# biotite-dev/springcraft

Measured on AMD Instinct MI355X. Metric: ANM modes/sec (Hessian build + full eigensolve), N=2000 C-alpha, higher is better.
Workload: dtype f64; 1 GPU; C3: N=2000 C-alpha ANM, HinsenForceField (no cutoff), full 6000x6000 eigensolve, all modes + vectors; parallelism=independent structures sharded over GPUs, no data-path collective

## Files before the change

### springcraft_amd/csrc/api.hip

```cpp
#include <algorithm>
#include <cmath>
#include <cstdarg>
#include <cstring>
#include <map>
#include <new>
#include <utility>

#include "common.h"
#include "host_logic.h"

int sc_set_error(sc_ctx* ctx, int code, const char* fmt, ...) {
  char buf[1024];
  va_list ap;
  va_start(ap, fmt);
  vsnprintf(buf, sizeof(buf), fmt, ap);
  va_end(ap);
  if (ctx) ctx->err = buf;
  return code;
}

static int reserve(sc_ctx* ctx, void*& buf, size_t& have, size_t bytes, bool collect_events = false) {
  if (bytes <= have) return SC_OK;
  if (buf) {
    SC_HIP(ctx, hipStreamSynchronize(ctx->stream));
// ... 326 lines not shown
}

const char* sc_last_error(sc_ctx* ctx) { return ctx ? ctx->err.c_str() : "null context"; }

int sc_host_alloc(size_t bytes, void** out) {
  if (!out || bytes == 0) return SC_ERR_INVALID_ARG;
  *out = nullptr;
  void* p = nullptr;
  if (hipHostMalloc(&p, bytes, hipHostMallocDefault) != hipSuccess || !p) {
    (void)hipGetLastError();
    return SC_ERR_NOMEM;
  }
  *out = p;
  return SC_OK;
}

int sc_host_free(void* p) {
  if (!p) return SC_OK;
  return hipHostFree(p) == hipSuccess ? SC_OK : SC_ERR_HIP;
}

int sc_ctx_synchronize(sc_ctx* ctx) {
  if (!ctx) return SC_ERR_INVALID_ARG;
  SC_HIP(ctx, hipSetDevice(ctx->device));
  SC_HIP(ctx, hipStreamSynchronize(ctx->stream));
  return sc_deferred_status(ctx);
}

int sc_device_info(sc_ctx* ctx, char* buf, size_t buflen) {
  if (!ctx || !buf || buflen == 0) return SC_ERR_INVALID_ARG;
  hipDeviceProp_t prop;
  SC_HIP(ctx, hipGetDeviceProperties(&prop, ctx->device));
  snprintf(buf, buflen, "%s %s, %d CUs, %.0f GiB", prop.gcnArchName, prop.name,
           prop.multiProcessorCount, (double)prop.totalGlobalMem / (1 << 30));
  return SC_OK;
}

int sc_ctx_set_profiling(sc_ctx* ctx, int enabled) {
  if (!ctx) return SC_ERR_INVALID_ARG;
  ctx->profiling = enabled != 0;
  return SC_OK;
}

int sc_last_eigh_timings(sc_ctx* ctx, double* out6) {
  if (!ctx || !out6) return SC_ERR_INVALID_ARG;
  for (int i = 0; i < 6; ++i) out6[i] = ctx->last_timings[i];
  return SC_OK;
}

int sc_last_eigh_phase_ms(sc_ctx* ctx, const char* name, double* ms) {
  if (!ctx || !name || !ms) return SC_ERR_INVALID_ARG;
  for (const auto& p : ctx->phases)
    if (p.first == name) { *ms = p.second; return SC_OK; }
  *ms = 0.0;
  return SC_ERR_INVALID_ARG;
}

int sc_ctx_get_counter(sc_ctx* ctx, const char* name, int64_t* value) {
  if (!ctx || !name || !value) return SC_ERR_INVALID_ARG;
  const std::string k(name);
  SC_HIP(ctx, hipSetDevice(ctx->device));
  SC_HIP(ctx, hipStreamSynchronize(ctx->stream));
  SC_TRY(sc_collect_events(ctx));
  int tmin = ctx->chase_tickets[0], tmax = ctx->chase_tickets[0];
  long long tsum = 0;
  for (int x = 0; x < std::max(1, std::min(8, ctx->chase_ctl_xcds)); ++x) {
    tmin = std::min(tmin, ctx->chase_tickets[x]);
    tmax = std::max(tmax, ctx->chase_tickets[x]);
    tsum += ctx->chase_tickets[x];
  }
  if (k == "chase_launches") *value = ctx->cnt_chase_launches;
  else if (k == "chase_pair_launches") *value = ctx->cnt_pair_launches;
  else if (k == "chase_pair_fallbacks") *value = ctx->cnt_pair_fallbacks;
  else if (k == "xcd_count") *value = ctx->nxcd;
  else if (k == "gemm3_launches") *value = ctx->cnt_gemm3_launches;
  else if (k == "symm3_launches") *value = ctx->cnt_symm3_launches;
  else if (k == "resident_launches") *value = ctx->cnt_resident_launches;
  else if (k == "resident_takeovers") *value = ctx->cnt_resident_takeovers;
  else if (k == "resident_rollcall_failures") *value = ctx->cnt_resident_rollcalls;
  else if (k == "resident_lost_waits") *value = ctx->cnt_resident_lost;
  else if (k == "resident_lost_at") *value = ctx->resident_lost_at;
  else if (k == "panel_coop_launches") *value = ctx->cnt_coop_launches;
  else if (k == "panel_coop_timeouts") *value = ctx->cnt_coop_timeouts;
  else if (k == "chase_timeouts") *value = ctx->cnt_chase_timeouts;
  else if (k == "chase_incomplete") *value = ctx->cnt_chase_incomplete;
  else if (k == "chase_resumed") *value = ctx->cnt_chase_resumed;
  else if (k == "chase_sweeps") *value = ctx->cnt_chase_sweeps;
  else if (k == "stepwise_chases") *value = ctx->cnt_stepwise_chases;
  else if (k == "chase_xcd_min") *value = tmin;
  else if (k == "chase_xcd_max") *value = tmax;
  else if (k == "chase_xcd_total") *value = tsum;
  else if (k == "chase_wait_matrix") *value = ctx->chase_wait[0];
  else if (k == "chase_wait_sweep") *value = ctx->chase_wait[1];
  else if (k == "chase_wait_task") *value = ctx->chase_wait[2];
  else { *value = 0; return SC_ERR_INVALID_ARG; }
  return SC_OK;
}

int sc_dbg_set_chase(sc_ctx* ctx, int mode, int give_up_after) {
  if (!ctx || mode < -1 || mode > 5 || give_up_after < 0) return SC_ERR_INVALID_ARG;
  ctx->chase_form = mode == 3 ? 1 : (mode == 4 ? 0 : (mode == 5 ? 2 : -1));
  if (mode > 2) mode = 2;
  ctx->chase_mode = mode;
  ctx->chase_give_up = give_up_after;
  if (mode >= 0) ctx->chase_ok = -1;
  return SC_OK;
}

int sc_dbg_set_panel_coop_fail(sc_ctx* ctx, int panel) {
  if (!ctx || panel < -1) return SC_ERR_INVALID_ARG;
  ctx->coop_fail_panel = panel;
  if (panel >= 0) ctx->coop_ok = -1;
  return SC_OK;
}

int sc_dbg_set_resident(sc_ctx* ctx, int mode, int hook, int workgroups) {
  if (!ctx || mode < -1 || mode > 1 || hook < 0 || workgroups < 0 || workgroups > 256) return SC_ERR_INVALID_ARG;
  ctx->resident_mode = mode;
  ctx->resident_hook = hook;
  ctx->resident_wgs = workgroups;
  if (mode != 0) { ctx->resident_ok = -1; ctx->resident_strikes = 0; }
  return SC_OK;
}

int sc_dbg_set_panel_coop(sc_ctx* ctx, int min_rows) {
  if (!ctx || min_rows < -1 || (min_rows > 0 && min_rows < 128)) return SC_ERR_INVALID_ARG;
  ctx->coop_min_rows = min_rows;
  if (min_rows != 0) ctx->coop_ok = -1;
  return SC_OK;
}

int sc_contacts(sc_ctx* ctx, const double* coord, int64_t n, const sc_ff_desc* ff,
                const sc_patch_desc* patch, int64_t* counts, int64_t* n_pairs) {
  SC_TRY(check_coord_args(ctx, coord, n));
  SC_TRY(check_ff(ctx, ff));
  SC_HIP(ctx, hipSetDevice(ctx->device));
  if (n_pairs) *n_pairs = 0;
  if (n == 0) return SC_OK;
  Staged st;
  Bump bump{};
  SC_TRY(stage_inputs(ctx, coord, n, ff, patch, nullptr, (size_t)n * 8 + 256, st, bump));
  int64_t* d_counts = bump.take<int64_t>((size_t)n);
  SC_TRY(launch_contact_counts(ctx, st.d_coord, n, st.ff_dev, st.has_patch ? &st.patch : nullptr, d_counts));
  std::vector<int64_t> h((size_t)n);
  SC_HIP(ctx, hipMemcpyAsync(h.data(), d_counts, (size_t)n * 8, hipMemcpyDeviceToHost, ctx->stream));
  SC_HIP(ctx, hipStreamSynchronize(ctx->stream));
  int64_t total = 0;
  for (int64_t i = 0; i < n; ++i) total += h[(size_t)i];
  if (counts) std::memcpy(counts, h.data(), (size_t)n * 8);
  if (n_pairs) *n_pairs = total;
  return SC_OK;
}

int sc_pairs(sc_ctx* ctx, const double* coord, int64_t n, const sc_ff_desc* ff,
             const sc_patch_desc* patch, int64_t capacity, int64_t* pairs, double* sq_dist,
             int64_t* n_pairs) {
  SC_TRY(check_coord_args(ctx, coord, n));
  SC_TRY(check_ff(ctx, ff));
  if (capacity < 0 || (capacity > 0 && !pairs))
    return sc_set_error(ctx, SC_ERR_INVALID_ARG, "pairs buffer is NULL");
  SC_HIP(ctx, hipSetDevice(ctx->device));
  if (n_pairs) *n_pairs = 0;
  if (n == 0) return SC_OK;
  Staged st;
  Bump bump{};
  const size_t extra = (size_t)(2 * n + 2) * 8 + (size_t)capacity * 24 + 2048;
// ... 1107 lines not shown
```

### springcraft_amd/csrc/common.h

```cpp
#pragma once

#include <hip/hip_runtime.h>

#include <cstdint>
#include <cstdio>
#include <map>
#include <mutex>
#include <string>
#include <utility>
#include <vector>

#include "../../include/springcraft_hip.h"

struct sc_ctx {
  int device = 0;
  hipStream_t stream = nullptr;
  bool own_stream = false;
  hipStream_t aux_stream = nullptr;
  std::vector<hipStream_t> side_streams;
  std::vector<hipEvent_t> side_joins;
  hipEvent_t aux_fork = nullptr, aux_join = nullptr;
  std::string err;
  int num_cus = 0;

  void* ws = nullptr;
  size_t ws_bytes = 0;
  void* scratch = nullptr;
  size_t scratch_bytes = 0;
  void* dc_aux = nullptr;
  size_t dc_aux_bytes = 0;
  void* pinv_ws = nullptr;
  size_t pinv_ws_bytes = 0;
  void* win_ws = nullptr;
  size_t win_ws_bytes = 0;
  void* modes_ws = nullptr;
  size_t modes_ws_bytes = 0;

  char* h_stage[2] = {nullptr, nullptr};
  size_t h_stage_bytes[2] = {0, 0}, h_stage_off[2] = {0, 0};
  hipEvent_t h_stage_done[2] = {nullptr, nullptr};
  bool h_stage_pending[2] = {false, false};
  int h_stage_cur = 0;
  unsigned long long* d_status = nullptr;

  int two_stage = -1;
  int chase_ok = -1;
  int chase_mode = -1, chase_give_up = 0;
  int chase_form = -1;
  int nxcd = 0;
  int pair_attr = -1;
  long long cnt_pair_fallbacks = 0;
  int gemm3_attr = -1;
  void* d_zeros = nullptr;
  long long cnt_symm3_launches = 0;
  bool gemm3_side_by_side = false;
  long long cnt_gemm3_launches = 0;
  int coop_attr = -1, coop_ok = -1;
  int coop_min_rows = -1;
  int coop_fail_panel = -1;
  int resident_ok = -1, resident_mode = -1, resident_hook = 0, resident_wgs = 0;
  long long cnt_resident_launches = 0, cnt_resident_takeovers = 0, cnt_resident_rollcalls = 0, cnt_resident_lost = 0;
  long long resident_lost_at = -1;
  int resident_strikes = 0;
  int* d_chase_ctl = nullptr;
  int* last_chase_ctl = nullptr;
  int chase_ctl_xcds = 8;
  long long cnt_coop_launches = 0, cnt_coop_timeouts = 0;
  long long cnt_chase_launches = 0, cnt_chase_timeouts = 0, cnt_chase_incomplete = 0, cnt_chase_resumed = 0,
            cnt_chase_sweeps = 0, cnt_stepwise_chases = 0, cnt_pair_launches = 0;
  int chase_tickets[8] = {0, 0, 0, 0, 0, 0, 0, 0};
  int chase_wait[3] = {-1, -1, -1};
  bool profiling = false;
  double last_timings[6] = {0, 0, 0, 0, 0, 0};
  std::vector<std::pair<std::string, double>> phases;
};

class PhaseTimer {
 public:
  PhaseTimer(sc_ctx* ctx, const char* name, hipStream_t st) : ctx_(ctx), name_(name), st_(st), on_(ctx->profiling) {}
  ~PhaseTimer() { for (hipEvent_t e : ev_) (void)hipEventDestroy(e); }
  void start() { mark(); }
  void stop() { mark(); }
  void finish() {
    if (!on_ || ev_.size() < 2) return;
    double total = 0.0;
    if (hipEventSynchronize(ev_.back()) != hipSuccess) return;
    for (size_t i = 0; i + 1 < ev_.size(); i += 2) {
      float ms = 0.f;
      if (hipEventElapsedTime(&ms, ev_[i], ev_[i + 1]) == hipSuccess) total += ms;
    }
    for (auto& p : ctx_->phases)
      if (p.first == name_) { p.second = total; return; }
    ctx_->phases.emplace_back(name_, total);
  }
 private:
  void mark() {
    if (!on_) return;
    hipEvent_t e = nullptr;
    if (hipEventCreate(&e) != hipSuccess) { on_ = false; return; }
    (void)hipEventRecord(e, st_);
    ev_.push_back(e);
  }
  sc_ctx* ctx_;
  std::string name_;
  hipStream_t st_;
  bool on_;
  std::vector<hipEvent_t> ev_;
};

template <int N>
struct ScopedEvents {
  hipEvent_t e[N];
  ScopedEvents() { for (auto& x : e) x = nullptr; }
  ~ScopedEvents() { for (auto& x : e) if (x) (void)hipEventDestroy(x); }
  ScopedEvents(const ScopedEvents&) = delete;
  ScopedEvents& operator=(const ScopedEvents&) = delete;
  hipEvent_t& operator[](int i) { return e[i]; }
  hipEvent_t* begin() { return e; }
  hipEvent_t* end() { return e + N; }
};

int sc_set_error(sc_ctx* ctx, int code, const char* fmt, ...);

#define SC_HIP(ctx, call)                                                              \
  do {                                                                                 \
    hipError_t e__ = (call);                                                           \
    if (e__ != hipSuccess)                                                             \
      return sc_set_error((ctx), e__ == hipErrorOutOfMemory ? SC_ERR_NOMEM : SC_ERR_HIP, \
                          "%s failed: %s (%s:%d)", #call, hipGetErrorString(e__),      \
                          __FILE__, __LINE__);                                         \
  } while (0)

#define SC_TRY(expr)            \
  do {                          \
    int rc__ = (expr);          \
    if (rc__ != SC_OK) return rc__; \
  } while (0)

int sc_reserve_ws(sc_ctx* ctx, size_t bytes);
int sc_reserve_scratch(sc_ctx* ctx, size_t bytes);
int sc_reserve_dc_aux(sc_ctx* ctx, size_t bytes);
int sc_reserve_pinv(sc_ctx* ctx, size_t bytes);
int sc_reserve_win(sc_ctx* ctx, size_t bytes);
int sc_reserve_modes(sc_ctx* ctx, size_t bytes);
int sc_aux_stream(sc_ctx* ctx);
int sc_side_streams(sc_ctx* ctx, int count);
int sc_stage_upload(sc_ctx* ctx, void* d_dst, const void* h_src, size_t bytes);
int sc_stage_end(sc_ctx* ctx);
constexpr int kSpStatusWords = 16;
constexpr int kChaseCtlInts = 32;
// ... 108 lines not shown
```

### springcraft_amd/csrc/sy2sb.hip

```cpp
#include <algorithm>
#include <vector>

#include "twostage_internal.h"

namespace {

constexpr int kEarly = (kIb + 2) / 2;

__global__ __launch_bounds__(256) void k_panel_qr(double* __restrict__ a_all, long long stride_a,
                                                  double* __restrict__ tri_all, TriLayout TL,
                                                  double* __restrict__ sb_all, SbLayout SL, int j0, int j, int nr,
                                                  int c_end) {
  constexpr int LD = kQrRows + 1;
  extern __shared__ __attribute__((aligned(16))) double sm[];
  const int c_lo = j > 0 ? j - 1 : 0;
  const int ncl = c_end - c_lo;
  double* P = sm;
  double* wv = sm + ncl * LD;
  double* vv = wv + kB;
  double* red = vv + kQrRows;
  __shared__ double s_scale, s_beta, s_tau;

  const int n = TL.n;
  const int r0 = j0 + kB, m = n - r0;
// ... 852 lines not shown
                                                       double* __restrict__ sb_all, SbLayout SL, int j0,
                                                       const int* __restrict__ ctl, unsigned long long* __restrict__ stats) {
  __shared__ double red[16 * 9];
  __shared__ double s_w[8];
  __shared__ double s_tau, s_beta, s_scale;
  const int mat = blockIdx.x;
  if (ctl[8 * mat] == 0) return;
  const int n = TL.n;
  const int r0 = j0 + kB, m = n - r0;
  double* A = a_all + (size_t)mat * stride_a;
  double* tri = tri_all + (size_t)mat * TL.slab;
  double* sb = sb_all + (size_t)mat * SL.slab;
  double* P = A + (size_t)j0 * n + r0;
  const int tid = threadIdx.x, lane = tid & 63, wv = tid >> 6;
  if (tid == 0) atomicAdd(stats + 5, 1ull);
  auto block_sum8 = [&](double (&a)[8], int cnt) {
    for (int i = 0; i < cnt; ++i) {
      const double t = wave_sum(a[i]);
      if (lane == 0) red[wv * 9 + i] = t;
    }
    __syncthreads();
    for (int i = 0; i < cnt; ++i) {
      double t = 0.0;
      for (int w = 0; w < 16; ++w) t += red[w * 9 + i];
      a[i] = t;
    }
    __syncthreads();
  };
  for (int j = 0; j < kB; ++j) {
    double* pj = P + (size_t)j * n;
    {
      double a[8] = {0, 0, 0, 0, 0, 0, 0, 0};
      for (int r = j + 1 + tid; r < m; r += 1024) a[0] += pj[r] * pj[r];
      block_sum8(a, 1);
      if (tid == 0) {
        const HH h = householder(pj[j], a[0]);
        s_tau = h.tau; s_beta = h.beta; s_scale = h.scale;
        tri[TL.tau + j0 + j] = h.tau;
      }
      __syncthreads();
    }
    const double tau = s_tau, scale = s_scale;
    for (int c0 = j + 1; c0 < kB; c0 += 8) {
      const int cnt = min(8, kB - c0);
      double a[8] = {0, 0, 0, 0, 0, 0, 0, 0};
      for (int r = j + 1 + tid; r < m; r += 1024) {
        const double x = pj[r];
        for (int i = 0; i < cnt; ++i) a[i] += x * P[(size_t)(c0 + i) * n + r];
      }
      block_sum8(a, cnt);
      if (tid < cnt) s_w[tid] = tau * (P[(size_t)(c0 + tid) * n + j] + scale * a[tid]);
      __syncthreads();
      for (int r = j + tid; r < m; r += 1024) {
        const double v = r > j ? scale * pj[r] : 1.0;
        for (int i = 0; i < cnt; ++i) P[(size_t)(c0 + i) * n + r] -= v * s_w[i];
      }
      __syncthreads();
    }
    for (int r = j + tid; r < m; r += 1024) pj[r] = r > j ? scale * pj[r] : s_beta;
    __syncthreads();
  }
  for (int c = 0; c < kB; ++c)
    for (int r = tid; r < m; r += 1024) {
      const double val = P[(size_t)c * n + r];
      const double v = r > c ? val : (r == c ? 1.0 : 0.0);
      sb[SL.vw + (size_t)c * n + r0 + r] = v;
      sb[SL.wv + (size_t)(kB + c) * n + r0 + r] = -v;
      sb[SL.xv + (size_t)(2 * kB + c) * n + r0 + r] = v;
    }
}

__global__ __launch_bounds__(256) void k_sum_xslices(double* __restrict__ sb_all, SbLayout SL, int r0) {
  const int n = SL.n, p = SL.symm_split;
  double* sb = sb_all + (size_t)blockIdx.z * SL.slab;
  const int which = blockIdx.y / kB, c = blockIdx.y % kB;
  const int r = r0 + blockIdx.x * 256 + threadIdx.x;
  if (r >= n) return;
  const double* src = sb + SL.xsplit + (size_t)which * p * n * kB + (size_t)c * n + r;
  double s = 0.0;
  for (int q = 0; q < p; ++q) s += src[(size_t)q * n * kB];
  sb[SL.xv + (size_t)(which * kB + c) * n + r] = s;
}

__global__ __launch_bounds__(256) void k_sum_p2(double* __restrict__ sb_all, SbLayout SL) {
  double* sb = sb_all + (size_t)blockIdx.y * SL.slab;
  const int i = blockIdx.x * 256 + threadIdx.x;
  double acc = 0.0;
#pragma unroll
  for (int sl = 0; sl < kSmallSplit; ++sl) acc += sb[SL.small2 + (size_t)sl * 2 * kB * kB + i];
  sb[SL.p2 + i] = acc;
}

__global__ __launch_bounds__(1024) void k_sb_small(const double* __restrict__ tri_all, TriLayout TL,
                                                   double* __restrict__ sb_all, SbLayout SL, int j0) {
  constexpr int LD = kB + 1;
  extern __shared__ __attribute__((aligned(16))) double sm[];
  double* G = sm;
  double* M1 = G + kB * LD;
  double* T = M1 + kB * LD;
  double* U = T + kB * LD;
  const double* tri = tri_all + (size_t)blockIdx.x * TL.slab;
  double* sb = sb_all + (size_t)blockIdx.x * SL.slab;
  const int tid = threadIdx.x, nthr = blockDim.x;
  const double* prod = sb + SL.small;
  const size_t slice = (size_t)kB * 3 * kB;
  for (int idx = tid; idx < kB * kB; idx += nthr) {
    const int i = idx & 63, jj = idx >> 6;
    double g = 0.0, x = 0.0;
#pragma unroll
    for (int s = 0; s < kSmallSplit; ++s) {
      const double* ps = prod + s * slice;
      x += ps[i + (size_t)jj * kB] + ps[i + (size_t)(kB + jj) * kB];
      g += ps[i + (size_t)(2 * kB + jj) * kB];
    }
    G[i * LD + jj] = g;
    M1[i * LD + jj] = x;
    T[i * LD + jj] = 0.0;
  }
  __syncthreads();
  if (tid < kB) {
    const int bb = tid >> 4, c = tid & 15, o = bb * 16;
    double x[16];
#pragma unroll
    for (int i = 15; i >= 0; --i) {
      double acc = (i == c) ? 1.0 : 0.0;
#pragma unroll
      for (int l = i + 1; l < 16; ++l) acc -= G[(o + i) * LD + o + l] * x[l];
      x[i] = i <= c ? tri[TL.tau + j0 + o + i] * acc : 0.0;
    }
#pragma unroll
    for (int i = 0; i < 16; ++i) T[(o + i) * LD + o + c] = x[i];
  }
  __syncthreads();
#pragma unroll
  for (int bs = 16; bs <= 32; bs *= 2) {
    const int npair = kB / (2 * bs);
    for (int idx = tid; idx < npair * bs * bs; idx += nthr) {
      const int pr = idx / (bs * bs), e = idx % (bs * bs), i = e / bs, jj = e % bs;
      const int o1 = pr * 2 * bs, o2 = o1 + bs;
      double acc = 0.0;
      for (int l = 0; l <= jj; ++l) acc += G[(o1 + i) * LD + o2 + l] * T[(o2 + l) * LD + o2 + jj];
      U[(o1 + i) * LD + o2 + jj] = acc;
    }
    __syncthreads();
    for (int idx = tid; idx < npair * bs * bs; idx += nthr) {
      const int pr = idx / (bs * bs), e = idx % (bs * bs), i = e / bs, jj = e % bs;
      const int o1 = pr * 2 * bs, o2 = o1 + bs;
      double acc = 0.0;
      for (int l = i; l < bs; ++l) acc += T[(o1 + i) * LD + o1 + l] * U[(o1 + l) * LD + o2 + jj];
      T[(o1 + i) * LD + o2 + jj] = -acc;
    }
    __syncthreads();
  }
  for (int idx = tid; idx < kB * kB; idx += nthr) {
    const int i = idx >> 6, jj = idx & 63;
    double s = 0.0;
    for (int l = 0; l <= jj; ++l) s += M1[i * LD + l] * T[l * LD + jj];
    U[i * LD + jj] = s;
  }
  __syncthreads();
  double* cm = sb + SL.cmat;
  for (int idx = tid; idx < kB * kB; idx += nthr) {
    const int i = idx & 63, jj = idx >> 6;
    double s = 0.0;
    for (int l = 0; l <= i; ++l) s += T[l * LD + i] * U[l * LD + jj];
    const double t = T[i * LD + jj];
    cm[i + (size_t)jj * 3 * kB] = t;
    cm[kB + i + (size_t)jj * 3 * kB] = t;
    cm[2 * kB + i + (size_t)jj * 3 * kB] = -0.5 * s;
  }
}

}


std::vector<GemmDesc> sb_stage1_records(int n, int batch, const std::vector<int>& role, double* d_a, long long stride_a,
                                        double* d_sb_ws, const SbLayout& SL) {
  const sc_host::TwoStageEnv& E = sc_host::two_stage_env();
  const int npanels = (int)role.size();
  std::vector<GemmDesc> h((size_t)npanels * kDescKinds * batch);
  for (int p = 0; p < npanels; ++p) {
    const int j0 = p * kB, r0 = j0 + kB, m = n - r0;
    const int rl = role[(size_t)p];
    const long long vw_w = rl == 2 ? 3 * kB : kB, wv_w = rl == 2 ? 2 * kB : 0;
    for (int b = 0; b < batch; ++b) {
      double* A = d_a + (size_t)b * stride_a;
      double* sb = d_sb_ws + (size_t)b * SL.slab;
      double* a22 = A + (size_t)r0 * n + r0;
      GemmDesc* g = &h[((size_t)p * batch + b) * kDescKinds];
      GemmDesc X1{};
      X1.a = a22; X1.sa_i = 1; X1.sa_k = n; X1.a_tri = 1;
      X1.b = sb + SL.xv + (size_t)2 * kB * n + r0; X1.sb_k = 1; X1.sb_j = n;
      X1.c = sb + SL.xv + r0; X1.ldc = n;
      X1.m = m; X1.n = kB; X1.k = m; X1.alpha = 1.0; X1.beta = 0.0;
      if (SL.symm_split > 1) {
        X1.c = sb + SL.xsplit + r0;
        X1.split_stride = (long long)n * kB;
      }
      g[0] = X1;
      GemmDesc X2 = X1;
      X2.sa_i = n; X2.sa_k = 1; X2.a_tri = 2;
      X2.c = sb + SL.xv + (size_t)kB * n + r0;
      if (SL.symm_split > 1) X2.c = sb + SL.xsplit + (size_t)SL.symm_split * n * kB + r0;
      g[1] = X2;
      GemmDesc P{};
      P.a = sb + SL.xv + (size_t)2 * kB * n + r0; P.sa_i = n; P.sa_k = 1;
      P.b = sb + SL.xv + r0; P.sb_k = 1; P.sb_j = n;
      P.c = sb + SL.small; P.ldc = kB;
      P.m = kB; P.n = 3 * kB; P.k = m; P.alpha = 1.0; P.beta = 0.0;
      P.split_stride = (long long)kB * 3 * kB;
      g[2] = P;
      GemmDesc W{};
      W.a = sb + SL.xv + r0; W.sa_i = 1; W.sa_k = n;
      W.b = sb + SL.cmat; W.sb_k = 1; W.sb_j = 3 * kB;
      W.c = sb + SL.vw + (size_t)vw_w * n + r0; W.ldc = n;
      W.m = m; W.n = kB; W.k = 3 * kB; W.alpha = 1.0; W.beta = 0.0;
      g[3] = W;
      W.c = sb + SL.wv + (size_t)wv_w * n + r0;
      W.alpha = -1.0;
      g[4] = W;
      GemmDesc R{};
      R.a = sb + SL.vw + r0; R.sa_i = 1; R.sa_k = n;
      R.b = sb + SL.wv + r0; R.sb_k = n; R.sb_j = 1;
      R.c = a22; R.ldc = n;
      R.m = m; R.n = m; R.k = rl == 2 ? 4 * kB : 2 * kB; R.alpha = 1.0; R.beta = 1.0;
      R.lower_only = sc_host::symm3_for(E, n) ? 2 : 1;
      g[5] = R;
      GemmDesc D = R;
      D.n = kB; D.k = 2 * kB;
      g[6] = D;
      GemmDesc Q{};
      Q.a = sb + SL.wv + r0; Q.sa_i = n; Q.sa_k = 1;
      Q.b = sb + SL.xv + (size_t)2 * kB * n + r0; Q.sb_k = 1; Q.sb_j = n;
      Q.c = sb + SL.small2; Q.ldc = 2 * kB;
      Q.m = 2 * kB; Q.n = kB; Q.k = m; Q.alpha = 1.0; Q.beta = 0.0;
      Q.split_stride = (long long)2 * kB * kB;
      g[7] = Q;
      GemmDesc Cr{};
      Cr.a = sb + SL.vw + r0; Cr.sa_i = 1; Cr.sa_k = n;
      Cr.b = sb + SL.p2; Cr.sb_k = 1; Cr.sb_j = 2 * kB;
      Cr.c = sb + SL.xv + r0; Cr.ldc = n;
      Cr.m = m; Cr.n = kB; Cr.k = 2 * kB; Cr.alpha = 1.0; Cr.beta = 1.0;
      g[8] = Cr;
    }
  }
  std::vector<GemmDesc> hs(h.size());
  for (int p = 0; p < npanels; ++p)
    for (int b = 0; b < batch; ++b) {
      const GemmDesc* g = &h[((size_t)p * batch + b) * kDescKinds];
      GemmDesc* o = &hs[(size_t)p * kDescKinds * batch];
      for (int kd = 0; kd < kDescKinds; ++kd) o[(size_t)kd * batch + b] = g[kd];
    }
  return hs;
}

struct PanelRun {
  sc_ctx* ctx;
  hipStream_t st;
  double* d_a; long long stride_a; int n, batch;
  double* d_tri_ws; const TriLayout& TL;
  double* d_sb_ws; const SbLayout& SL;
  const GemmDesc* d_descs;
  const std::vector<int>& role;
  sc_host::CoopPlan coop;
  v4i* coop_recs;
  int* coop_ctl;
  bool use_symm3;
  int symm3_nb_min;
  SbTimers& t;
};

static int run_panel(const PanelRun& R, int p, int lo, int hi, hipStream_t ps, bool timed) {
  using sc_host::PanelQr;
  const sc_host::TwoStageEnv& E = sc_host::two_stage_env();
  sc_ctx* ctx = R.ctx;
  const TriLayout& TL = R.TL;
  const SbLayout& SL = R.SL;
  const int n = R.n, batch = R.batch;
  const long long stride_a = R.stride_a;
  struct StreamScope {
    sc_ctx* c; hipStream_t old;
    StreamScope(sc_ctx* c_, hipStream_t s) : c(c_), old(c_->stream) { c->stream = s; }
    ~StreamScope() { c->stream = old; }
  } scope(ctx, ps);
  const int nb = hi - lo;
  const int rl = R.role[(size_t)p];
  double* a_h = R.d_a + (size_t)lo * stride_a;
  double* tri_h = R.d_tri_ws + (size_t)lo * TL.slab;
  double* sb_h = R.d_sb_ws + (size_t)lo * SL.slab;
  const int j0 = p * kB, r0 = j0 + kB, m = n - r0;
  const int nr = std::min(kB, m - 1);
  const int nchunks = (m + kQrRows - 1) / kQrRows;
  const dim3 qgrid((unsigned)nchunks, (unsigned)nb);
  SbLayout SQ = SL;
  if (rl == 2) { SQ.vw += (long long)2 * kB * n; SQ.wv += (long long)2 * kB * n; }
  if (timed) R.t.qr.start();
  const sc_host::PanelQrForm F = sc_host::panel_qr_form(E, R.coop, R.coop_recs != nullptr, m, nb, ps == R.st);
  switch (F.kind) {
    case PanelQr::Coop: {
      const int coop_g = F.coop_g;
      if (p == ctx->coop_fail_panel) SC_HIP(ctx, hipMemsetAsync(R.coop_ctl + 8 * lo, 1, sizeof(int) * 8 * nb, ps));
      hipLaunchKernelGGL(k_panel_coop, dim3((unsigned)coop_g, (unsigned)nb), dim3(kCoopRows), kCoopLdsBytes, ps, a_h, stride_a,
                         tri_h, TL, sb_h, SQ, j0, coop_g, R.coop_recs + (size_t)lo * coop_recs_per_matrix(coop_g),
                         R.coop_ctl + 8 * lo, (p + 1) * 128);
      hipLaunchKernelGGL(k_panel_serial, dim3((unsigned)nb), dim3(1024), 0, ps, a_h, stride_a, tri_h, TL, sb_h, SQ, j0,
                         (const int*)(R.coop_ctl + 8 * lo), ctx->d_status);
      ++ctx->cnt_coop_launches;
      break;
    }
    case PanelQr::Wg1024: {
      const size_t lds_wg = sizeof(double) * (size_t)(2 * kWgWaves * 8 + 16 + 8 + 8 * kB + kWgWaves * kB * 8);
      const dim3 g1((unsigned)nb), b1((unsigned)kWgThreads);
      if (F.ru == 1) hipLaunchKernelGGL((k_panel_wg<1, 8>), g1, b1, lds_wg, ps, a_h, stride_a, tri_h, TL, sb_h, SQ, j0);
      else if (F.ru == 2) hipLaunchKernelGGL((k_panel_wg<2, 8>), g1, b1, lds_wg, ps, a_h, stride_a, tri_h, TL, sb_h, SQ, j0);
      else if (F.ru == 3) hipLaunchKernelGGL((k_panel_wg<3, 4>), g1, b1, lds_wg, ps, a_h, stride_a, tri_h, TL, sb_h, SQ, j0);
      else hipLaunchKernelGGL((k_panel_wg<4, 2>), g1, b1, lds_wg, ps, a_h, stride_a, tri_h, TL, sb_h, SQ, j0);
      break;
    }
    case PanelQr::Wg512: {
      constexpr int kW = 512 / 64;
      const size_t lds_wg = sizeof(double) * (size_t)(2 * kW * 8 + 16 + 8 + 8 * kB + kW * kB * 8);
      const dim3 g1((unsigned)nb), b1(512u);
      if (F.ru == 10) hipLaunchKernelGGL((k_panel_wg<10, 1, 512>), g1, b1, lds_wg, ps, a_h, stride_a, tri_h, TL, sb_h, SQ, j0);
      else hipLaunchKernelGGL((k_panel_wg<12, 1, 512>), g1, b1, lds_wg, ps, a_h, stride_a, tri_h, TL, sb_h, SQ, j0);
      break;
    }
    case PanelQr::Blocked: {
      const size_t lds_qr_blk = sizeof(double) * ((size_t)(kIb + 1) * (kQrRows + 1) + kB + kQrRows + 4 * kB);
      const size_t lds_blk_a = sizeof(double) * ((size_t)kB * (kQrRows + 1) + kQrRows + 8 * kB);
      const size_t lds_blk_b = sizeof(double) * ((size_t)kB * (kQrRows + 1) + kIb * kB + 4 * kB);
      hipLaunchKernelGGL(k_panel_qr, qgrid, dim3(256), lds_qr_blk, ps, a_h, stride_a, tri_h, TL, sb_h, SQ, j0, 0, nr, kIb);
      for (int c0 = 0; c0 < kB; c0 += kIb) {
        for (int j = c0 + 1; j < c0 + kIb; ++j)
          hipLaunchKernelGGL(k_panel_qr, qgrid, dim3(256), lds_qr_blk, ps, a_h, stride_a, tri_h, TL, sb_h, SQ, j0, j, nr,
                             c0 + kIb);
        const size_t cut = sizeof(double) * (size_t)c0 * (kQrRows + 1);
        hipLaunchKernelGGL(k_pqr_blk_a, qgrid, dim3(256), lds_blk_a - cut, ps, a_h, stride_a, tri_h, TL, sb_h, SQ, j0, c0);
        if (c0 + kIb < kB)
          hipLaunchKernelGGL(k_pqr_blk_b, qgrid, dim3(256), lds_blk_b - cut, ps, a_h, stride_a, tri_h, TL, sb_h, SQ, j0, c0);
      }
      break;
    }
    case PanelQr::Unblocked: {
      const size_t lds_qr = sizeof(double) * ((size_t)kB * (kQrRows + 1) + kB + kQrRows + 4 * kB);
      for (int j = 0; j <= nr; ++j)
        hipLaunchKernelGGL(k_panel_qr, qgrid, dim3(256), lds_qr, ps, a_h, stride_a, tri_h, TL, sb_h, SQ, j0, j, nr, kB);
      break;
    }
  }
  if (timed) R.t.qr.stop();
  const GemmDesc* g = R.d_descs + (size_t)p * kDescKinds * batch;
  if (timed) R.t.symm.start();
  if (R.use_symm3 && symm3_would_take(ctx, R.symm3_nb_min, m, SL.symm_split, true) &&
      launch_symm3(ctx, g + lo, nb, m, SL.symm_split, true, true) == SC_OK) {
    if (SL.symm_split > 1)
      hipLaunchKernelGGL(k_sum_xslices, dim3((unsigned)((m + 255) / 256), kB, (unsigned)nb), dim3(256), 0, ps, sb_h, SL, r0);
  } else {
    SC_TRY(launch_gemm_f64(ctx, g + lo, nb, m, kB, kGemmTile, SL.symm_split, false, true, kGemmAmBk));
    SC_TRY(launch_gemm_f64(ctx, g + batch + lo, nb, m, kB, kGemmTile, SL.symm_split, false, true, kGemmAkBk));
    if (SL.symm_split > 1)
      hipLaunchKernelGGL(k_sum_xslices, dim3((unsigned)((m + 255) / 256), 2 * kB, (unsigned)nb), dim3(256), 0, ps, sb_h, SL, r0);
  }
  if (rl == 2) {
    SC_TRY(launch_gemm_f64(ctx, g + 7 * batch + lo, nb, 2 * kB, kB, kGemmTile, kSmallSplit, false, false, kGemmAkBk));
    hipLaunchKernelGGL(k_sum_p2, dim3((unsigned)(2 * kB * kB / 256), (unsigned)nb), dim3(256), 0, ps, sb_h, SL);
    SC_TRY(launch_gemm_f64(ctx, g + 8 * batch + lo, nb, m, kB, kGemmTile, 1, false, false, kGemmAmBk));
  }
  if (timed) R.t.symm.stop();
  SC_TRY(launch_gemm_f64(ctx, g + 2 * batch + lo, nb, kB, 3 * kB, kGemmTile, kSmallSplit, false, false, kGemmAkBk));
  const size_t lds_small = sizeof(double) * 4 * kB * (kB + 1);
  hipLaunchKernelGGL(k_sb_small, dim3((unsigned)nb), dim3(1024), lds_small, ps, tri_h, TL, sb_h, SL, j0);
  if (nb == batch) {
    SC_TRY(launch_gemm_f64(ctx, g + 3 * batch, 2 * batch, m, kB, kGemmTile, 1, false, false, kGemmAmBk));
  } else {
    SC_TRY(launch_gemm_f64(ctx, g + 3 * batch + lo, nb, m, kB, kGemmTile, 1, false, false, kGemmAmBk));
    SC_TRY(launch_gemm_f64(ctx, g + 4 * batch + lo, nb, m, kB, kGemmTile, 1, false, false, kGemmAmBk));
  }
  if (timed) R.t.syr2k.start();
  if (rl == 1)
    SC_TRY(launch_gemm_f64(ctx, g + 6 * batch + lo, nb, m, kB, kGemmTile, 1, false, false, kGemmAmBn));
  else
    if (launch_gemm3_uniform(ctx, g + 5 * batch + lo, nb, m, m, rl == 2 ? 4 * kB : 2 * kB, kGemmAmBn, R.use_symm3 ? 2 : 1, 1.0, 1.0,
                             (n & 1) == 0 && (r0 & 1) == 0) != SC_OK)
      SC_TRY(launch_gemm_f64(ctx, g + 5 * batch + lo, nb, m, m, kGemmTile, 1, false, false, kGemmAmBn, true));
  if (timed) R.t.syr2k.stop();
  return SC_OK;
}

int sb_stage1(sc_ctx* ctx, double* d_a, long long stride_a, int n, int batch, double* d_tri_ws, const TriLayout& TL,
              double* d_sb_ws, const SbLayout& SL, const GemmDesc* d_descs, const std::vector<int>& role, bool prof,
              SbTimers& timers) {
  const sc_host::TwoStageEnv& E = sc_host::two_stage_env();
  hipStream_t st = ctx->stream;
  const int npanels = (int)role.size();

  for (int b = 0; b < batch; ++b)
    SC_HIP(ctx, hipMemsetAsync(d_tri_ws + (size_t)b * TL.slab + TL.tau, 0, sizeof(double) * n, st));

  const int s1_parts = sc_host::stage1_parts(E, batch, prof);
  const sc_host::CoopPlan coop = sc_host::coop_plan(E, n, batch, ctx->num_cus, prof, ctx->coop_min_rows, ctx->coop_ok);
  v4i* coop_recs = nullptr;
  int* coop_ctl = nullptr;
  if (coop.ask) {
    if (ctx->coop_attr < 0)
      ctx->coop_attr = hipFuncSetAttribute(reinterpret_cast<const void*>(&k_panel_coop),
                                           hipFuncAttributeMaxDynamicSharedMemorySize, (int)kCoopLdsBytes) == hipSuccess;
    if (ctx->coop_attr == 1 && coop.nb_max >= 1) {
      const size_t rec_bytes = (size_t)batch * coop_recs_per_matrix(coop.gmax) * sizeof(v4i);
      const size_t ctl_bytes = align_up((size_t)batch * 8 * sizeof(int), 256);
      SC_TRY(sc_reserve_dc_aux(ctx, ctl_bytes + rec_bytes));
      coop_ctl = reinterpret_cast<int*>(ctx->dc_aux);
      coop_recs = reinterpret_cast<v4i*>(reinterpret_cast<char*>(ctx->dc_aux) + ctl_bytes);
      SC_HIP(ctx, hipMemsetAsync(ctx->dc_aux, 0, ctl_bytes + rec_bytes, st));
    }
  }
  const bool use_symm3 = sc_host::symm3_for(E, n);
  if (use_symm3)
    for (int b = 0; b < batch; ++b)
      SC_HIP(ctx, hipMemsetAsync(d_sb_ws + (size_t)b * SL.slab + SL.xv + (size_t)kB * n, 0, sizeof(double) * (size_t)kB * n, st));
  const PanelRun R{ctx, st, d_a, stride_a, n, batch, d_tri_ws, TL, d_sb_ws, SL, d_descs, role, coop, coop_recs, coop_ctl,
                   use_symm3, std::max(1, batch / s1_parts), timers};
  if (s1_parts > 1) {
    struct SideBySide {
      sc_ctx* c;
      explicit SideBySide(sc_ctx* c_) : c(c_) { c->gemm3_side_by_side = true; }
      ~SideBySide() { c->gemm3_side_by_side = false; }
    } side_by_side(ctx);
    SC_TRY(sc_aux_stream(ctx));
    SC_TRY(sc_side_streams(ctx, s1_parts - 1));
    SC_HIP(ctx, hipEventRecord(ctx->aux_fork, st));
    for (int q = 1; q < s1_parts; ++q) SC_HIP(ctx, hipStreamWaitEvent(ctx->side_streams[q - 1], ctx->aux_fork, 0));
    int rc_parts = SC_OK;
    for (int p = 0; p < npanels && rc_parts == SC_OK; ++p)
      for (int q = 0; q < s1_parts && rc_parts == SC_OK; ++q) {
        const int lo = (int)((long long)batch * q / s1_parts), hi = (int)((long long)batch * (q + 1) / s1_parts);
        rc_parts = run_panel(R, p, lo, hi, q == 0 ? st : ctx->side_streams[q - 1], q == 0);
      }
    for (int q = 1; q < s1_parts; ++q) {
      SC_HIP(ctx, hipEventRecord(ctx->side_joins[q - 1], ctx->side_streams[q - 1]));
      SC_HIP(ctx, hipStreamWaitEvent(st, ctx->side_joins[q - 1], 0));
    }
    SC_TRY(rc_parts);
  } else {
    for (int p = 0; p < npanels; ++p) SC_TRY(run_panel(R, p, 0, batch, st, true));
  }
  SC_HIP(ctx, hipGetLastError());
  return SC_OK;
}
```

### springcraft_amd/csrc/twostage.hip

```cpp
#include <algorithm>
#include <vector>

#include "twostage_internal.h"

size_t sb_slab_doubles(int n, int batch, SbLayout* out) {
  SbLayout L{};
  L.n = n;
  long long off = 0;
  auto take = [&](long long cnt) { long long o = off; off += (cnt + 31) / 32 * 32; return o; };
  const int nchunk = (n + kQrRows - 1) / kQrRows + 1;
  L.vw = take((long long)n * 4 * kB);
  L.wv = take((long long)n * 4 * kB);
  L.xv = take((long long)n * 3 * kB);
  L.symm_split = sc_host::symm_split_for(sc_host::two_stage_env(), n, batch);
  L.xsplit = L.symm_split > 1 ? take((long long)2 * L.symm_split * n * kB) : 0;
  L.qrpart = take((long long)2 * nchunk * kB);
  L.qrpiv = take(2 * (kB + 8));
  L.qrpart8 = take((long long)nchunk * kIb * kB);
  L.small = take((long long)kSmallSplit * kB * 3 * kB);
  L.cmat = take(3 * kB * kB);
  L.small2 = take((long long)kSmallSplit * 2 * kB * kB);
  L.p2 = take(2 * kB * kB);
  L.ab = take((long long)kLdab * n);
  const int nsweep = std::max(n - 2, 0);
  L.ngroups = (nsweep + kG - 1) / kG;
  long long ndia = 0;
  for (int S = 0; S < L.ngroups; ++S) {
    const int len = (n - 1 - S * kG + kB - 1) / kB;
    ndia += len;
  }
  L.ndia = ndia;
  L.vd = take(ndia * kDiaSize);
  L.frag = take(ndia * kFragDoubles);
  L.tau2 = take(ndia * kG);
  L.slab = off;
  if (out) *out = L;
  return (size_t)off;
}

int sb_desc_count(int n, int batch) {
  const int npanels = n / kB + 1;
  return npanels * kDescKinds * batch;
}

int sytrd_2stage_batched(sc_ctx* ctx, double* d_a, long long stride_a, int n, int batch, double* d_tri_ws,
                         const TriLayout& TL, double* d_sb_ws, const SbLayout& SL, int* d_dia_off,
                         GemmDesc* d_descs, float* ms_stage1, float* ms_stage2, double* d_band_copy) {
  hipStream_t st = ctx->stream;
  ScopedEvents<3> ev;
  const bool prof = ctx->profiling && ms_stage1 && ms_stage2;
  if (prof) {
    for (auto& e : ev) SC_HIP(ctx, hipEventCreate(&e));
    SC_HIP(ctx, hipEventRecord(ev[0], st));
  }

  const std::vector<int> role = sc_host::panel_roles(sc_host::two_stage_env(), n);
  const std::vector<GemmDesc> hs = sb_stage1_records(n, batch, role, d_a, stride_a, d_sb_ws, SL);
  if (!hs.empty()) SC_TRY(sc_stage_upload(ctx, d_descs, hs.data(), hs.size() * sizeof(GemmDesc)));
  const std::vector<int> doff = dia_offsets(n);
  SC_TRY(sc_stage_upload(ctx, d_dia_off, doff.data(), doff.size() * sizeof(int)));

  SbTimers timers(ctx, st);
  SC_TRY(sb_stage1(ctx, d_a, stride_a, n, batch, d_tri_ws, TL, d_sb_ws, SL, d_descs, role, prof, timers));
  if (prof) SC_HIP(ctx, hipEventRecord(ev[1], st));
  SC_TRY(sb_stage2(ctx, d_a, stride_a, n, batch, d_tri_ws, TL, d_sb_ws, SL, d_band_copy, timers));
  if (prof) {
    SC_HIP(ctx, hipEventRecord(ev[2], st));
    SC_HIP(ctx, hipEventSynchronize(ev[2]));
    SC_HIP(ctx, hipEventElapsedTime(ms_stage1, ev[0], ev[1]));
    SC_HIP(ctx, hipEventElapsedTime(ms_stage2, ev[1], ev[2]));
  }
  timers.finish();
  return SC_OK;
}

int sb_band_width() { return kB; }

extern "C" int sc_dbg_two_stage(sc_ctx* ctx, const double* a, int n, double* band_out, double* d_out, double* e_out) {
  if (!ctx || !a || n < 4 * kB) return SC_ERR_INVALID_ARG;
  SC_HIP(ctx, hipSetDevice(ctx->device));
  TriLayout TL{};
  TL.n = n; TL.nb = kB;
  TL.d = 0; TL.e = n; TL.tau = 2 * (long long)n; TL.slab = 3 * (long long)n + 64;
  SbLayout SL;
  const size_t sbd = sb_slab_doubles(n, 1, &SL);
  double *d_a = nullptr, *d_tri = nullptr, *d_sb = nullptr, *d_band = nullptr;
  int* d_off = nullptr;
  GemmDesc* d_desc = nullptr;
  SC_HIP(ctx, hipMalloc(&d_a, sizeof(double) * (size_t)n * n));
  SC_HIP(ctx, hipMalloc(&d_tri, sizeof(double) * TL.slab));
  SC_HIP(ctx, hipMalloc(&d_sb, sizeof(double) * sbd));
  SC_HIP(ctx, hipMalloc(&d_band, sizeof(double) * kLdab * n));
  SC_HIP(ctx, hipMalloc(&d_off, sizeof(int) * (n / 64 + 8)));
  SC_HIP(ctx, hipMalloc(&d_desc, sizeof(GemmDesc) * sb_desc_count(n, 1)));
  SC_HIP(ctx, hipMemcpyAsync(d_a, a, sizeof(double) * (size_t)n * n, hipMemcpyHostToDevice, ctx->stream));
  int rc = mirror_lower_batched(ctx, d_a, (long long)n * n, n, 1);
  if (rc == SC_OK)
    rc = sytrd_2stage_batched(ctx, d_a, (long long)n * n, n, 1, d_tri, TL, d_sb, SL, d_off, d_desc, nullptr, nullptr,
                              d_band);
  if (rc == SC_OK) {
    (void)hipMemcpy(band_out, d_band, sizeof(double) * kLdab * n, hipMemcpyDeviceToHost);
    (void)hipMemcpy(d_out, d_tri + TL.d, sizeof(double) * n, hipMemcpyDeviceToHost);
    (void)hipMemcpy(e_out, d_tri + TL.e, sizeof(double) * n, hipMemcpyDeviceToHost);
  }
  (void)hipFree(d_a); (void)hipFree(d_tri); (void)hipFree(d_sb); (void)hipFree(d_band); (void)hipFree(d_off);
// ... 4 lines not shown
```

### springcraft_amd/csrc/twostage_policy.h

```cpp
#pragma once
#include <algorithm>
#include <cstddef>
#include <cstdlib>
#include <vector>

#if defined(__HIPCC__)
#define SC_POLICY_HD __host__ __device__
#else
#define SC_POLICY_HD
#endif

namespace sc_host {

constexpr int kBand = 64;
constexpr int kWgRows1024 = 4 * 1024;
constexpr int kWgRows512 = 12 * 512;
constexpr int kCoopRows = 256;
constexpr int kCoopMaxG = 128;
constexpr int kEarlyRing = 8;

static inline size_t policy_align_up(size_t x, size_t a) { return (x + a - 1) / a * a; }

SC_POLICY_HD inline int chase_len(int n, int s) { return (n - 1 - s + kBand - 1) / kBand; }

struct TwoStageEnv {
  int symm3 = 1;
  int symm_split = 0;
  bool panel_pairs = true;
  bool qr_blocked = true;
  int qr_wg = -1;
  int qr_coop = 1;
  int qr_coop_min = 0;
  int stage1_streams = 0;
  int bulge_persistent = 1;
  int bulge_pair = -1;
  long long bulge_pair_max = 6000;
  int bulge_spread = -1;
  bool bulge_no_early = false;
  int bulge_streams = 0;
  int bulge_burst = 32;
  int bt2_wave = -1;
  int bt2_nw = 0;
};

static inline TwoStageEnv read_two_stage_env() {
  TwoStageEnv E;
  auto num = [](const char* name, int unset) { const char* e = getenv(name); return e ? atoi(e) : unset; };
  E.symm3 = num("SPRINGCRAFT_SYMM3", 1);
  E.symm_split = num("SPRINGCRAFT_SYMM_SPLIT", 0);
  E.panel_pairs = num("SPRINGCRAFT_PANEL_PAIRS", 1) != 0;
  E.qr_blocked = getenv("SPRINGCRAFT_QR_UNBLOCKED") == nullptr;
  E.qr_wg = num("SPRINGCRAFT_QR_WG", -1);
  E.qr_coop = num("SPRINGCRAFT_QR_COOP", 1);
  if (const char* e = getenv("SPRINGCRAFT_QR_COOP_MIN")) E.qr_coop_min = std::max(2 * kBand, atoi(e));
  E.stage1_streams = num("SPRINGCRAFT_STAGE1_STREAMS", 0);
  E.bulge_persistent = num("SPRINGCRAFT_BULGE_PERSISTENT", 1);
  E.bulge_pair = num("SPRINGCRAFT_BULGE_PAIR", -1);
  if (const char* e = getenv("SPRINGCRAFT_BULGE_PAIR_MAX")) E.bulge_pair_max = atoll(e);
  E.bulge_spread = num("SPRINGCRAFT_BULGE_SPREAD", -1);
  E.bulge_no_early = getenv("SPRINGCRAFT_BULGE_NO_EARLY") != nullptr;
  E.bulge_streams = num("SPRINGCRAFT_BULGE_STREAMS", 0);
  E.bulge_burst = std::max(1, num("SPRINGCRAFT_BULGE_BURST", 32));
  E.bt2_wave = num("SPRINGCRAFT_BT2_WAVE", -1);
  E.bt2_nw = num("SPRINGCRAFT_BT2_NW", 0);
  return E;
}
inline const TwoStageEnv& two_stage_env() {
  static const TwoStageEnv E = read_two_stage_env();
  return E;
}


static inline int stage1_parts(const TwoStageEnv& E, int batch, bool profiled) {
  const int want = E.stage1_streams > 0 ? E.stage1_streams : ((batch >= 32 && !profiled) ? 2 : 1);
  return std::max(1, std::min(want, std::min(batch, 4)));
}

static inline int panel_count(int n) {
  int npanels = 0;
  while (n - (npanels + 1) * kBand >= 2) ++npanels;
  return npanels;
}
static inline std::vector<int> panel_roles(const TwoStageEnv& E, int n) {
  const int npanels = panel_count(n);
  std::vector<int> role((size_t)npanels, 0);
  if (E.panel_pairs)
    for (int p = 0; p + 1 < npanels;) {
      const int m2 = n - (p + 2) * kBand;
      if (m2 >= 4 * kBand) { role[(size_t)p] = 1; role[(size_t)p + 1] = 2; p += 2; }
      else ++p;
    }
  return role;
}

static inline bool symm3_for(const TwoStageEnv& E, int n) { return E.symm3 != 0 && n >= 512 && (n & 1) == 0; }

static inline int symm_split_for(const TwoStageEnv& E, int n, int batch) {
  if (E.symm_split >= 1) return std::min(E.symm_split, 16);
  if (symm3_for(E, n)) {
    const long long items = (long long)((n + 127) / 128) * (batch >= 32 ? batch / 2 : batch);
    if (items >= 768) return 1;
    return (int)std::min<long long>(16, (1536 + items - 1) / items);
  }
  const long long tiles = (long long)batch * ((n + 63) / 64);
  if (tiles >= 1024 || n < 2048) return 1;
  const long long s0 = std::min<long long>(6, (2048 + tiles - 1) / tiles);
  return s0 >= 6 ? 9 : (s0 == 4 ? 5 : (int)s0);
}

struct CoopPlan {
  bool ask;
  int nb_max;
  int min_few;
  int min_many;
  int budget;
  int gmax;
};
static inline CoopPlan coop_plan(const TwoStageEnv& E, int n, int batch, int num_cus, bool profiled, int coop_min_rows,
                                 int coop_ok) {
  CoopPlan C{};
  C.min_few = coop_min_rows > 0 ? coop_min_rows : (E.qr_coop_min > 0 ? E.qr_coop_min : 300);
  C.min_many = coop_min_rows > 0 ? coop_min_rows : (E.qr_coop_min > 0 ? E.qr_coop_min : kWgRows512 + 1);
  C.budget = num_cus * 3 / 4;
  C.gmax = (std::max(n - kBand, 1) + kCoopRows - 1) / kCoopRows;
  C.ask = (coop_min_rows > 0 || (coop_min_rows < 0 && E.qr_coop != 0)) && coop_ok != 0 &&
          n - kBand >= std::min(C.min_few, C.min_many) && C.gmax <= kCoopMaxG && stage1_parts(E, batch, profiled) == 1;
  C.nb_max = std::min(batch, C.budget / C.gmax);
  return C;
}

enum class PanelQr {
  Coop,
  Wg1024,
  Wg512,
  Blocked,
  Unblocked,
};
struct PanelQrForm {
  PanelQr kind;
  int ru, cu;
  int coop_g;
};
static inline PanelQrForm panel_qr_form(const TwoStageEnv& E, const CoopPlan& C, bool have_recs, int m, int nb,
                                        bool main_stream) {
  PanelQrForm F{PanelQr::Unblocked, 0, 0, (m + kCoopRows - 1) / kCoopRows};
  const bool full = std::min(kBand, m - 1) == kBand;
  const bool use_wg = full && m <= kWgRows1024 && E.qr_wg != 0;
  const bool use_wg512 = full && !use_wg && m <= kWgRows512 && E.qr_wg != 0 && E.qr_wg != 1 && nb >= 4;
  const bool use_coop = have_recs && full && m >= (nb < 4 ? C.min_few : C.min_many) && nb * F.coop_g <= C.budget && main_stream;
  if (use_coop) {
    F.kind = PanelQr::Coop;
  } else if (use_wg) {
    F.kind = PanelQr::Wg1024;
    const int ru = (m + 1023) / 1024;
    F.ru = ru <= 1 ? 1 : std::min(ru, 4);
    F.cu = ru <= 2 ? 8 : (ru == 3 ? 4 : 2);
  } else if (use_wg512) {
    F.kind = PanelQr::Wg512;
    F.ru = (m + 511) / 512 <= 10 ? 10 : 12;
    F.cu = 1;
  } else if (full && E.qr_blocked) {
    F.kind = PanelQr::Blocked;
  }
  return F;
}


enum class ChaseForm {
  Stepwise,
  Sweep,
  Spread,
  Pair,
};
static inline ChaseForm chase_form_for(const TwoStageEnv& E, int n, int batch, int nxcd, int num_cus, bool pair_attr,
// ... 68 lines not shown
```

Measured before the change: 179,500 modes/s.

## Generalize deferred panel pairing to groups of up to four panels

Generalizes the sy2sb panel scheme so trailing-matrix rank updates can be deferred across groups of 2 or 4 panels instead of only pairs. Role encoding, workspace sizing, the correction GEMMs and the final syr2k update are all parameterized by group position. Larger groups would cut the number of full trailing syr2k passes, at the cost of larger k and extra correction work per panel. The default group stays 2, so the default path should behave the same as before apart from the more general indexing.

```diff
diff --git a/springcraft_amd/csrc/api.hip b/springcraft_amd/csrc/api.hip
--- a/springcraft_amd/csrc/api.hip
+++ b/springcraft_amd/csrc/api.hip
@@ -432,6 +432,7 @@
   else if (k == "resident_lost_at") *value = ctx->resident_lost_at;
   else if (k == "panel_coop_launches") *value = ctx->cnt_coop_launches;
   else if (k == "panel_coop_timeouts") *value = ctx->cnt_coop_timeouts;
+  else if (k == "panel_groups4") *value = ctx->cnt_panel_groups4;
   else if (k == "chase_timeouts") *value = ctx->cnt_chase_timeouts;
   else if (k == "chase_incomplete") *value = ctx->cnt_chase_incomplete;
   else if (k == "chase_resumed") *value = ctx->cnt_chase_resumed;
diff --git a/springcraft_amd/csrc/common.h b/springcraft_amd/csrc/common.h
--- a/springcraft_amd/csrc/common.h
+++ b/springcraft_amd/csrc/common.h
@@ -66,6 +66,7 @@
   int* last_chase_ctl = nullptr;
   int chase_ctl_xcds = 8;
   long long cnt_coop_launches = 0, cnt_coop_timeouts = 0;
+  long long cnt_panel_groups4 = 0;
   long long cnt_chase_launches = 0, cnt_chase_timeouts = 0, cnt_chase_incomplete = 0, cnt_chase_resumed = 0,
             cnt_chase_sweeps = 0, cnt_stepwise_chases = 0, cnt_pair_launches = 0;
   int chase_tickets[8] = {0, 0, 0, 0, 0, 0, 0, 0};
diff --git a/springcraft_amd/csrc/sy2sb.hip b/springcraft_amd/csrc/sy2sb.hip
--- a/springcraft_amd/csrc/sy2sb.hip
+++ b/springcraft_amd/csrc/sy2sb.hip
@@ -958,12 +958,12 @@
   sb[SL.xv + (size_t)(which * kB + c) * n + r] = s;
 }
 
-__global__ __launch_bounds__(256) void k_sum_p2(double* __restrict__ sb_all, SbLayout SL) {
+__global__ __launch_bounds__(256) void k_sum_p2(double* __restrict__ sb_all, SbLayout SL, int count) {
   double* sb = sb_all + (size_t)blockIdx.y * SL.slab;
   const int i = blockIdx.x * 256 + threadIdx.x;
   double acc = 0.0;
 #pragma unroll
-  for (int sl = 0; sl < kSmallSplit; ++sl) acc += sb[SL.small2 + (size_t)sl * 2 * kB * kB + i];
+  for (int sl = 0; sl < kSmallSplit; ++sl) acc += sb[SL.small2 + (size_t)sl * count + i];
   sb[SL.p2 + i] = acc;
 }
 
@@ -1058,7 +1058,9 @@
   for (int p = 0; p < npanels; ++p) {
     const int j0 = p * kB, r0 = j0 + kB, m = n - r0;
     const int rl = role[(size_t)p];
-    const long long vw_w = rl == 2 ? 3 * kB : kB, wv_w = rl == 2 ? 2 * kB : 0;
+    const int jg = std::max(1, sc_host::role_pos(rl));
+    const int kprev = 2 * kB * (jg - 1);
+    const long long vw_w = kprev + kB, wv_w = kprev;
     for (int b = 0; b < batch; ++b) {
       double* A = d_a + (size_t)b * stride_a;
       double* sb = d_sb_ws + (size_t)b * SL.slab;
@@ -1099,24 +1101,25 @@
       R.a = sb + SL.vw + r0; R.sa_i = 1; R.sa_k = n;
       R.b = sb + SL.wv + r0; R.sb_k = n; R.sb_j = 1;
       R.c = a22; R.ldc = n;
-      R.m = m; R.n = m; R.k = rl == 2 ? 4 * kB : 2 * kB; R.alpha = 1.0; R.beta = 1.0;
+      R.m = m; R.n = m; R.k = kprev + 2 * kB; R.alpha = 1.0; R.beta = 1.0;
       R.lower_only = sc_host::symm3_for(E, n) ? 2 : 1;
       g[5] = R;
       GemmDesc D = R;
-      D.n = kB; D.k = 2 * kB;
+      D.n = kB;
       g[6] = D;
+      const int kq = std::max(kprev, 2 * kB);
       GemmDesc Q{};
       Q.a = sb + SL.wv + r0; Q.sa_i = n; Q.sa_k = 1;
       Q.b = sb + SL.xv + (size_t)2 * kB * n + r0; Q.sb_k = 1; Q.sb_j = n;
-      Q.c = sb + SL.small2; Q.ldc = 2 * kB;
-      Q.m = 2 * kB; Q.n = kB; Q.k = m; Q.alpha = 1.0; Q.beta = 0.0;
-      Q.split_stride = (long long)2 * kB * kB;
+      Q.c = sb + SL.small2; Q.ldc = kq;
+      Q.m = kq; Q.n = kB; Q.k = m; Q.alpha = 1.0; Q.beta = 0.0;
+      Q.split_stride = (long long)kq * kB;
       g[7] = Q;
       GemmDesc Cr{};
       Cr.a = sb + SL.vw + r0; Cr.sa_i = 1; Cr.sa_k = n;
-      Cr.b = sb + SL.p2; Cr.sb_k = 1; Cr.sb_j = 2 * kB;
+      Cr.b = sb + SL.p2; Cr.sb_k = 1; Cr.sb_j = kq;
       Cr.c = sb + SL.xv + r0; Cr.ldc = n;
-      Cr.m = m; Cr.n = kB; Cr.k = 2 * kB; Cr.alpha = 1.0; Cr.beta = 1.0;
+      Cr.m = m; Cr.n = kB; Cr.k = kq; Cr.alpha = 1.0; Cr.beta = 1.0;
       g[8] = Cr;
     }
   }
@@ -1168,8 +1171,10 @@
   const int nr = std::min(kB, m - 1);
   const int nchunks = (m + kQrRows - 1) / kQrRows;
   const dim3 qgrid((unsigned)nchunks, (unsigned)nb);
+  const int jg = std::max(1, sc_host::role_pos(rl));
+  const int kprev = 2 * kB * (jg - 1);
   SbLayout SQ = SL;
-  if (rl == 2) { SQ.vw += (long long)2 * kB * n; SQ.wv += (long long)2 * kB * n; }
+  SQ.vw += (long long)kprev * n; SQ.wv += (long long)kprev * n;
   if (timed) R.t.qr.start();
   const sc_host::PanelQrForm F = sc_host::panel_qr_form(E, R.coop, R.coop_recs != nullptr, m, nb, ps == R.st);
   switch (F.kind) {
@@ -1237,9 +1242,9 @@
     if (SL.symm_split > 1)
       hipLaunchKernelGGL(k_sum_xslices, dim3((unsigned)((m + 255) / 256), 2 * kB, (unsigned)nb), dim3(256), 0, ps, sb_h, SL, r0);
   }
-  if (rl == 2) {
-    SC_TRY(launch_gemm_f64(ctx, g + 7 * batch + lo, nb, 2 * kB, kB, kGemmTile, kSmallSplit, false, false, kGemmAkBk));
-    hipLaunchKernelGGL(k_sum_p2, dim3((unsigned)(2 * kB * kB / 256), (unsigned)nb), dim3(256), 0, ps, sb_h, SL);
+  if (jg >= 2) {
+    SC_TRY(launch_gemm_f64(ctx, g + 7 * batch + lo, nb, kprev, kB, kGemmTile, kSmallSplit, false, false, kGemmAkBk));
+    hipLaunchKernelGGL(k_sum_p2, dim3((unsigned)(kprev * kB / 256), (unsigned)nb), dim3(256), 0, ps, sb_h, SL, kprev * kB);
     SC_TRY(launch_gemm_f64(ctx, g + 8 * batch + lo, nb, m, kB, kGemmTile, 1, false, false, kGemmAmBk));
   }
   if (timed) R.t.symm.stop();
@@ -1253,10 +1258,10 @@
     SC_TRY(launch_gemm_f64(ctx, g + 4 * batch + lo, nb, m, kB, kGemmTile, 1, false, false, kGemmAmBk));
   }
   if (timed) R.t.syr2k.start();
-  if (rl == 1)
+  if (!sc_host::role_closes(rl))
     SC_TRY(launch_gemm_f64(ctx, g + 6 * batch + lo, nb, m, kB, kGemmTile, 1, false, false, kGemmAmBn));
   else
-    if (launch_gemm3_uniform(ctx, g + 5 * batch + lo, nb, m, m, rl == 2 ? 4 * kB : 2 * kB, kGemmAmBn, R.use_symm3 ? 2 : 1, 1.0, 1.0,
+    if (launch_gemm3_uniform(ctx, g + 5 * batch + lo, nb, m, m, kprev + 2 * kB, kGemmAmBn, R.use_symm3 ? 2 : 1, 1.0, 1.0,
                              (n & 1) == 0 && (r0 & 1) == 0) != SC_OK)
       SC_TRY(launch_gemm_f64(ctx, g + 5 * batch + lo, nb, m, m, kGemmTile, 1, false, false, kGemmAmBn, true));
   if (timed) R.t.syr2k.stop();
@@ -1269,6 +1274,7 @@
   const sc_host::TwoStageEnv& E = sc_host::two_stage_env();
   hipStream_t st = ctx->stream;
   const int npanels = (int)role.size();
+  for (int rl : role) ctx->cnt_panel_groups4 += rl == sc_host::kMaxPanelGroup;
 
   for (int b = 0; b < batch; ++b)
     SC_HIP(ctx, hipMemsetAsync(d_tri_ws + (size_t)b * TL.slab + TL.tau, 0, sizeof(double) * n, st));
diff --git a/springcraft_amd/csrc/twostage.hip b/springcraft_amd/csrc/twostage.hip
--- a/springcraft_amd/csrc/twostage.hip
+++ b/springcraft_amd/csrc/twostage.hip
@@ -9,8 +9,9 @@
   long long off = 0;
   auto take = [&](long long cnt) { long long o = off; off += (cnt + 31) / 32 * 32; return o; };
   const int nchunk = (n + kQrRows - 1) / kQrRows + 1;
-  L.vw = take((long long)n * 4 * kB);
-  L.wv = take((long long)n * 4 * kB);
+  const int gblocks = 2 * std::max(2, sc_host::panel_group_for(sc_host::two_stage_env()));
+  L.vw = take((long long)n * gblocks * kB);
+  L.wv = take((long long)n * gblocks * kB);
   L.xv = take((long long)n * 3 * kB);
   L.symm_split = sc_host::symm_split_for(sc_host::two_stage_env(), n, batch);
   L.xsplit = L.symm_split > 1 ? take((long long)2 * L.symm_split * n * kB) : 0;
@@ -19,8 +20,8 @@
   L.qrpart8 = take((long long)nchunk * kIb * kB);
   L.small = take((long long)kSmallSplit * kB * 3 * kB);
   L.cmat = take(3 * kB * kB);
-  L.small2 = take((long long)kSmallSplit * 2 * kB * kB);
-  L.p2 = take(2 * kB * kB);
+  L.small2 = take((long long)kSmallSplit * (gblocks - 2) * kB * kB);
+  L.p2 = take((gblocks - 2) * kB * kB);
   L.ab = take((long long)kLdab * n);
   const int nsweep = std::max(n - 2, 0);
   L.ngroups = (nsweep + kG - 1) / kG;
diff --git a/springcraft_amd/csrc/twostage_policy.h b/springcraft_amd/csrc/twostage_policy.h
--- a/springcraft_amd/csrc/twostage_policy.h
+++ b/springcraft_amd/csrc/twostage_policy.h
@@ -27,6 +27,7 @@
   int symm3 = 1;
   int symm_split = 0;
   bool panel_pairs = true;
+  int panel_group = 2;
   bool qr_blocked = true;
   int qr_wg = -1;
   int qr_coop = 1;
@@ -49,6 +50,7 @@
   E.symm3 = num("SPRINGCRAFT_SYMM3", 1);
   E.symm_split = num("SPRINGCRAFT_SYMM_SPLIT", 0);
   E.panel_pairs = num("SPRINGCRAFT_PANEL_PAIRS", 1) != 0;
+  E.panel_group = num("SPRINGCRAFT_PANEL_GROUP", E.panel_group);
   E.qr_blocked = getenv("SPRINGCRAFT_QR_UNBLOCKED") == nullptr;
   E.qr_wg = num("SPRINGCRAFT_QR_WG", -1);
   E.qr_coop = num("SPRINGCRAFT_QR_COOP", 1);
@@ -81,15 +83,25 @@
   while (n - (npanels + 1) * kBand >= 2) ++npanels;
   return npanels;
 }
+constexpr int kRoleMore = 16;
+constexpr int kMaxPanelGroup = 4;
+SC_POLICY_HD inline int role_pos(int role) { return role & (kRoleMore - 1); }
+SC_POLICY_HD inline bool role_closes(int role) { return role == 0 || (role_pos(role) >= 2 && !(role & kRoleMore)); }
+static inline int panel_group_for(const TwoStageEnv& E) {
+  if (!E.panel_pairs || E.panel_group < 2) return 1;
+  return E.panel_group >= 4 ? 4 : 2;
+}
 static inline std::vector<int> panel_roles(const TwoStageEnv& E, int n) {
   const int npanels = panel_count(n);
   std::vector<int> role((size_t)npanels, 0);
-  if (E.panel_pairs)
-    for (int p = 0; p + 1 < npanels;) {
-      const int m2 = n - (p + 2) * kBand;
-      if (m2 >= 4 * kBand) { role[(size_t)p] = 1; role[(size_t)p + 1] = 2; p += 2; }
-      else ++p;
-    }
+  const int gmax = panel_group_for(E);
+  for (int p = 0; p < npanels;) {
+    int g = gmax;
+    while (g > 1 && !(p + g <= npanels && n - (p + g) * kBand >= 4 * kBand)) g /= 2;
+    if (g > 1)
+      for (int j = 1; j <= g; ++j) role[(size_t)(p + j - 1)] = j | ((j >= 2 && j < g) ? kRoleMore : 0);
+    p += g;
+  }
   return role;
 }
 
```

Measured after the change: 179,600 modes/s, median of 6. Within noise of the previous version (+0.1%).
